# GuanRunwei/Achelous

Measured on AMD Instinct MI355X. Metric: frames/sec (whole node) EN-GDF-PN-S0 320x320+512pts bs64 @1/2/4/8 GPU, higher is better.
Workload: dtype bf16; 1 GPU; EN-GDF-PN-S0 forward + decode + NMS, 320x320 image + radar map, 512 points, batch 64 per GPU, all 5 heads, seeded random weights; radar_map=256 occupied cells per frame of 102 400 (SURVEY 8d: real maps are > 99 % zeros), global_batch=64, parallelism=batch-sharded x1, launches_per_forward=113

## Files before the change

achelous_amd/csrc/engine_impl.h:

```cpp
#pragma once
#include "engine.h"

#include <algorithm>
#include <cmath>
#include <cstring>

#include "k_dechead.h"
#include "k_csphead.h"
#include "k_upchain.h"
#include "k_detect.h"
#include "k_conv3.h"
#include "k_gemm.h"
#include "k_ghost.h"
#include "k_headdw.h"
#include "k_mlp.h"
#include "k_mlpband.h"
#include "k_mv2.h"
#include "k_mvit.h"
#include "k_nhwc.h"
#include "k_points.h"
#include "k_pn2.h"
#include "k_prepost.h"
#include "k_radar.h"
#include <functional>
#include "k_sdta.h"
#include "k_xca.h"
#include "k_xcaframe.h"

namespace ach {

#define ACH_HIP_CHECK(expr)                                                                               \
    do {                                                                                                  \
        hipError_t e_ = (expr);                                                                           \
        if (e_ != hipSuccess) throw AchError{ACH_ERR_DEVICE, std::string(#expr) + ": " + hipGetErrorString(e_)}; \
    } while (0)

static inline long round_up(long v, long m) { return (v + m - 1) / m * m; }

template <class T>
class Engine final : public EngineBase {
    using S = Store<T>;
    static constexpr int VEC = S::VEC;
    static constexpr int KC = 4 * VEC;
    static constexpr bool H16E = is_h16<T>::value;
    using IOB = typename std::conditional<std::is_same<T, f16_t>::value, bf16_t, T>::type;
    bool io_alt() const { return std::is_same<T, f16_t>::value && io_bf16; }

public:
    explicit Engine(const ach_config& c) : EngineBase(c) {}

    struct A {
        T* p = nullptr; int B = 0, H = 0, W = 0, C = 0; long ld = 0;
        long rows() const { return long(B) * H * W; }
        A slice(int c0, int c) const { A s = *this; s.p = p + c0; s.C = c; return s; }
    };
    struct Pl {
        T* p = nullptr; int B = 0, C = 0, H = 0, W = 0;
    };
    struct Lin { std::vector<float> w, b; int N = 0, K = 0; };

    A alloc(int B, int H, int W, int C) {
        A a; a.B = B; a.H = H; a.W = W; a.C = C; a.ld = round_up(C, 8);
        a.p = static_cast<T*>(aalloc(size_t(a.rows()) * a.ld * sizeof(T)));
        note_region(a.p, size_t(a.rows()) * a.ld * sizeof(T));
        return a;
    }
    A alloc_ld(int B, int H, int W, int C, long ld) {
        A a; a.B = B; a.H = H; a.W = W; a.C = C; a.ld = ld;
        a.p = static_cast<T*>(aalloc(size_t(a.rows()) * a.ld * sizeof(T)));
        note_region(a.p, size_t(a.rows()) * a.ld * sizeof(T));
        return a;
    }
    Pl alloc_pl(int B, int C, int H, int W) {
        Pl a; a.B = B; a.C = C; a.H = H; a.W = W;
        a.p = static_cast<T*>(aalloc(size_t(B) * C * H * W * sizeof(T)));
        note_region(a.p, size_t(B) * C * H * W * sizeof(T));
        return a;
    }
    float* alloc_f32(size_t n) { return static_cast<float*>(aalloc(n * sizeof(float))); }

    T* up_T(const std::vector<float>& v) {
        T* d = static_cast<T*>(walloc(v.size() * sizeof(T)));
        if (!measuring) {
            std::vector<T> h(v.size());
            for (size_t i = 0; i < v.size(); ++i) S::st(&h[i], v[i]);
            ACH_HIP_CHECK(hipMemcpy(d, h.data(), h.size() * sizeof(T), hipMemcpyHostToDevice));
        }
        return d;
    }
    void tap(const std::string& name, const A& a) {
        TapInfo t; t.ptr = a.p; t.kind = 0; t.B = a.B; t.H = a.H; t.W = a.W; t.C = a.C; t.ld = a.ld; add_tap(name, t);
    }
    void tap(const std::string& name, const Pl& a) {
        TapInfo t; t.ptr = a.p; t.kind = 1; t.B = a.B; t.H = a.H; t.W = a.W; t.C = a.C; add_tap(name, t);
    }

    Lin lin(const std::string& wkey, const std::string& bkey) const {
        const HostTensor& w = W(wkey);
        if (w.shape.size() < 2) throw AchError{ACH_ERR_MISSING_KEY, "not a matrix: " + wkey};
        Lin l; l.N = int(w.shape[0]); l.K = int(w.numel() / w.shape[0]);
        l.w = w.data;
        if (!bkey.empty() && hasW(bkey)) { l.b = W(bkey).data; if (int(l.b.size()) != l.N) throw AchError{ACH_ERR_MISSING_KEY, "bias shape: " + bkey}; }
        else l.b.assign(size_t(l.N), 0.f);
        return l;
    }
    void bn_coeffs(const std::string& pfx, double eps, std::vector<float>& scale, std::vector<float>& shift) const {
        const auto& g = W(pfx + ".weight").data; const auto& b = W(pfx + ".bias").data;
        const auto& m = W(pfx + ".running_mean").data; const auto& v = W(pfx + ".running_var").data;
        scale.resize(g.size()); shift.resize(g.size());
        for (size_t i = 0; i < g.size(); ++i) {
            const double s = double(g[i]) / std::sqrt(double(v[i]) + eps);
            scale[i] = float(s); shift[i] = float(double(b[i]) - double(m[i]) * s);
        }
    }
    void fold_bn(Lin& l, const std::string& pfx, double eps) const {
        std::vector<float> sc, sh; bn_coeffs(pfx, eps, sc, sh);
        if (int(sc.size()) != l.N) throw AchError{ACH_ERR_MISSING_KEY, "BatchNorm width mismatch at " + pfx};
        for (int n = 0; n < l.N; ++n) {
            for (int k = 0; k < l.K; ++k) l.w[size_t(n) * l.K + k] *= sc[n];
            l.b[n] = l.b[n] * sc[n] + sh[n];
        }
    }
    void fold_ln_in(Lin& l, const std::string& pfx) const {
        const auto& lw = W(pfx + ".weight").data; const auto& lb = W(pfx + ".bias").data;
        if (int(lw.size()) != l.K) throw AchError{ACH_ERR_MISSING_KEY, "LayerNorm width mismatch at " + pfx};
        for (int n = 0; n < l.N; ++n) {
            double acc = l.b[n];
            for (int k = 0; k < l.K; ++k) { acc += double(l.w[size_t(n) * l.K + k]) * lb[k]; l.w[size_t(n) * l.K + k] *= lw[k]; }
            l.b[n] = float(acc);
        }
    }
    void fold_scale_out(Lin& l, const std::vector<float>& g) const {
        for (int n = 0; n < l.N; ++n) { for (int k = 0; k < l.K; ++k) l.w[size_t(n) * l.K + k] *= g[n]; l.b[n] *= g[n]; }
    }

    std::vector<std::function<void()>> post_plan;
    struct Packed { T* w = nullptr; float* b = nullptr; int N = 0, K = 0, NT = 1, nchunks = 0, ksteps = 0; long group_elems = 0; };
    static int pick_nt(int N) { return N <= 16 ? 1 : (N <= 32 ? 2 : 4); }
    Packed pack_shape(int N, int K) const {
        Packed p; p.N = N; p.K = K; p.NT = pick_nt(N);
        p.nchunks = cdiv(N, 16 * p.NT); p.ksteps = cdiv(K, KC);
        p.group_elems = long(p.nchunks) * p.ksteps * p.NT * 64 * VEC;
        return p;
    }
    Packed pack(const Lin& l) {
        Packed p = pack_shape(l.N, l.K);
        std::vector<float> blob(size_t(p.group_elems), 0.f);
        if (!measuring)
            for (int n = 0; n < l.N; ++n)
                for (int k = 0; k < l.K; ++k) blob[size_t(wfrag_offset(n, k, p.NT, p.ksteps, VEC))] = l.w[size_t(n) * l.K + k];
        p.w = up_T(blob);
        p.b = up_f32(l.b);
        return p;
    }

    struct GemmOpt {
        int act = ACT_NONE; bool ln = false; float ln_eps = 0.f;
        bool ln_tap = false;
        const A* residual = nullptr;
        int conv_k = 0, conv_s = 1, conv_p = 0, Hin = 0, Win = 0, Cin = 0, Ho = 0, Wo = 0;
        int Creal = 0;
        void** ydyn = nullptr; int out_nchw = 0, HW = 0, Ctot = 0, coff = 0;
        int groups = 1; long w_group_stride = 0;
        const T* w_override = nullptr;
    };
    void gemm(const std::string& name, const T* Xp, long ldx, long M, const Packed& pk, T* Yp, long ldy, const GemmOpt& o) {
        GemmParams g;
        std::memset(&g, 0, sizeof(g));
        g.X = Xp; g.ldx = ldx; g.conv_k = o.conv_k; g.conv_s = o.conv_s; g.conv_p = o.conv_p; g.Hin = o.Hin; g.Win = o.Win; g.Cin = o.Cin; g.Ho = o.Ho; g.Wo = o.Wo;
        g.W = o.w_override ? o.w_override : pk.w; g.w_group_stride = o.w_group_stride;
        g.bias = pk.b; g.bias_group_stride = 0;
        g.Y = Yp; g.ldy = ldy;
        g.R = o.residual ? o.residual->p : nullptr; g.ldr = o.residual ? o.residual->ld : 0;
        g.groups = o.groups; g.M_per_group = int(M / o.groups);
        g.K = pk.K; g.N = pk.N; g.nchunks = pk.nchunks; g.ksteps = pk.ksteps;
        g.act = o.act; g.ln = o.ln_tap ? 2 : (o.ln ? 1 : 0); g.ln_eps = o.ln_eps;
        if (o.ln_tap && (o.conv_k != 2 || pk.NT != 4 || o.groups != 1 || batching || o.Cin % VEC != 0)) throw AchError{ACH_ERR_INVALID, name + ": per-tap LayerNorm needs a 2x2 conv with more than 32 outputs"};
        g.out_nchw = (o.out_nchw && io_alt()) ? 2 : o.out_nchw; g.HW = o.HW; g.Ctot = o.Ctot; g.coff = o.coff;
        g.vec_store = (ldy % 8 == 0 && (!o.residual || o.residual->ld % 8 == 0)) ? 1 : 0;
        if (ldx % VEC != 0) throw AchError{ACH_ERR_INVALID, name + ": activation row stride not 16-byte aligned"};
        if (o.conv_k > 0 && (o.Cin % VEC != 0 || pk.K != o.conv_k * o.conv_k * o.Cin)) throw AchError{ACH_ERR_UNSUPPORTED, name + ": conv channel count not 16-byte aligned"};
        const long kTargetBlocks = gemm_blocks > 0 ? gemm_blocks : 1024;
        int P = (!batching && pk.K >= 1024 && o.groups == 1 && gemm_rows > 1) ? gemm_rows : 1;
        while (P > 1 && cdivl(g.M_per_group, 64L * P) * pk.nchunks < 512) P >>= 1;
        const long row_blocks = cdivl(g.M_per_group, 64L * P) * g.groups;
        int zsplit = int(std::min<long>(pk.nchunks, std::max<long>(1, cdivl(kTargetBlocks, row_blocks))));
        g.chunks_per_block = cdiv(pk.nchunks, zsplit);
        const int NT = pk.NT;
        void** ydyn = o.ydyn;
        const double esz = double(sizeof(T));
        const double px_in = o.conv_k > 0 ? double(M) / (double(o.Ho) * o.Wo) * o.Hin * o.Win : 0.0;
        const double in_bytes = o.conv_k > 0 ? px_in * (o.Creal ? o.Creal : o.Cin) * esz : double(M) * pk.K * esz;
        const double rest = double(M) * pk.N * esz + (o.residual ? double(M) * pk.N * esz : 0.0)
                            + double(pk.group_elems) * esz * (o.w_group_stride ? o.groups : 1);
        const double bytes = in_bytes + rest;
        const double lbytes = (o.conv_k > 0 ? px_in * o.Cin * esz : in_bytes) + rest;
        if (batching) {
            if (g.groups != 1 || P != 1) throw AchError{ACH_ERR_INVALID, name + ": batched GEMMs must be ungrouped"};
            BatchJob j; j.kind = 0; j.name = name; j.g = g; j.NT = NT; j.ydyn = ydyn; j.bytes = bytes; j.flops = 2.0 * double(M) * (o.conv_k > 0 && o.Creal ? double(o.conv_k * o.conv_k * o.Creal) : double(pk.K)) * pk.N;
            batch_jobs.push_back(j);
            return;
        }
        add_op(name, [g, NT, P, ydyn](hipStream_t s) mutable {
            if (ydyn) g.Y = *ydyn;
            launch_gemm<T>(g, NT, P, s);
        }, bytes, 2.0 * double(M) * (o.conv_k > 0 && o.Creal ? double(o.conv_k * o.conv_k * o.Creal) : double(pk.K)) * pk.N, lbytes);
    }
    struct BatchJob { int kind = 0; std::string name; GemmParams g; int NT = 1; void** ydyn = nullptr; DwParams d; int ks = 0; double bytes = 0, flops = 0; HeadDwJob hj; int shared_in = 0; };
    bool batching = false;
    std::vector<BatchJob> batch_jobs;
    void flush_batch(int levels, int per_level) {
        batching = false;
        if (int(batch_jobs.size()) != levels * per_level || levels > 3) throw AchError{ACH_ERR_INVALID, "head batching: unexpected job count"};
        for (int st = 0; st < per_level; ++st) {
            const BatchJob& j0 = batch_jobs[size_t(st)];
            double bytes = 0, flops = 0;
            const std::string name = j0.name + "+levels";
            if (j0.kind == 0) {
                GemmJobs m;
                std::memset(&m, 0, sizeof(m));
                m.n = levels;
                unsigned gx = 1, gz = 1;
                void** yd[3] = {nullptr, nullptr, nullptr};
                for (int l = 0; l < levels; ++l) {
                    const BatchJob& j = batch_jobs[size_t(l * per_level + st)];
                    if (j.kind != 0 || j.NT != j0.NT) throw AchError{ACH_ERR_INVALID, "head batching: layer shapes differ across levels"};
                    m.p[l] = j.g;
                    m.nbx[l] = unsigned(cdivl(j.g.M_per_group, 64L));
                    m.nbz[l] = unsigned(cdiv(j.g.nchunks, j.g.chunks_per_block));
                    gx = std::max(gx, m.nbx[l]); gz = std::max(gz, m.nbz[l]);
                    yd[l] = j.ydyn; bytes += j.bytes; flops += j.flops;
                }
                const dim3 grid(gx, unsigned(levels), gz), block(256);
                const int NT = j0.NT;
                void** y0 = yd[0]; void** y1 = yd[1]; void** y2 = yd[2];
                add_op(name, [m, grid, block, NT, y0, y1, y2](hipStream_t s) mutable {
                    if (y0) m.p[0].Y = *y0;
                    if (y1) m.p[1].Y = *y1;
                    if (y2) m.p[2].Y = *y2;
                    if (NT == 1) ACH_LAUNCH((gemm_multi_kernel<T, 1>), grid, block, s, m);
                    else if (NT == 2) ACH_LAUNCH((gemm_multi_kernel<T, 2>), grid, block, s, m);
                    else ACH_LAUNCH((gemm_multi_kernel<T, 4>), grid, block, s, m);
                }, bytes, flops);
            } else if (j0.kind == 2) {
                HeadDwParams hp;
                std::memset(&hp, 0, sizeof(hp));
                hp.njobs = levels; hp.shared_in = j0.shared_in; hp.dbg = head_fuse_dbg;
                int wg = 0;
                for (int l = 0; l < levels; ++l) {
                    const BatchJob& j = batch_jobs[size_t(l * per_level + st)];
                    if (j.kind != 2 || j.shared_in != j0.shared_in) throw AchError{ACH_ERR_INVALID, "head batching: fused layers differ across levels"};
                    hp.job[l] = j.hj; hp.job[l].wg0 = wg;
                    hp.B = j.d.B;
                    wg += 2 * j.hj.bands * j.d.B;
                    bytes += j.bytes; flops += j.flops;
                }
                const dim3 grid(static_cast<unsigned>(wg)), block(HDW_THREADS);
                if constexpr (H16E)
                    add_op(name, [hp, grid, block](hipStream_t s) { ACH_LAUNCH((headdw_kernel<T>), grid, block, s, hp); }, bytes, flops);
                else throw AchError{ACH_ERR_INVALID, "head batching: the fused layer exists for 16-bit storage only"};
            } else {
                DwJobs m;
                std::memset(&m, 0, sizeof(m));
                m.n = levels;
                unsigned gx = 1;
                for (int l = 0; l < levels; ++l) {
                    const BatchJob& j = batch_jobs[size_t(l * per_level + st)];
                    if (j.kind != 1 || j.ks != 5 || j.d.stride != 1) throw AchError{ACH_ERR_INVALID, "head batching: depthwise shapes differ across levels"};
                    m.p[l] = j.d;
                    m.nbx[l] = unsigned(cdivl(long(j.d.B) * j.d.Ho * cdiv(j.d.Wo, 4) * (j.d.C / 4), 256));
                    gx = std::max(gx, m.nbx[l]);
                    bytes += j.bytes;
                }
                const dim3 grid(gx, unsigned(levels)), block(256);
                add_op(name, [m, grid, block](hipStream_t s) { ACH_LAUNCH((dwconv_strip_multi_kernel<T, 5, 4>), grid, block, s, m); }, bytes, 0);
            }
        }
        batch_jobs.clear();
    }
    void gemm(const std::string& name, const A& X, const Packed& pk, const A& Y, const GemmOpt& o = GemmOpt()) {
        gemm(name, X.p, X.ld, X.rows(), pk, Y.p, Y.ld, o);
    }

    void dwconv(const std::string& name, const A& X, const A* X2, const std::string& wkey, const std::string& bkey,
                const std::string& bnpfx, double bneps, int ks, int stride, int act, const A& Y) {
        const HostTensor& w = W(wkey);
        const int C = X.C;
        if (w.shape[0] != C || w.numel() != long(C) * ks * ks) throw AchError{ACH_ERR_MISSING_KEY, "depthwise weight shape: " + wkey};
        if (C % 4) throw AchError{ACH_ERR_UNSUPPORTED, name + ": depthwise channel count must be a multiple of 4"};
        std::vector<float> wt(size_t(ks) * ks * C), bias(size_t(C), 0.f), sc(size_t(C), 1.f), sh(size_t(C), 0.f);
        if (!bkey.empty()) bias = W(bkey).data;
        if (!bnpfx.empty()) bn_coeffs(bnpfx, bneps, sc, sh);
        for (int c = 0; c < C; ++c) {
            for (int t = 0; t < ks * ks; ++t) wt[size_t(t) * C + c] = w.data[size_t(c) * ks * ks + t] * sc[c];
            bias[c] = bias[c] * sc[c] + sh[c];
        }
        if (double(X.rows()) * double(std::max(X.ld, X2 ? X2->ld : 0L)) * sizeof(T) >= 2147483648.0)
            throw AchError{ACH_ERR_UNSUPPORTED, name + ": depthwise input of 2 GiB or more (batch too large for one plan)"};
        DwParams p;
        std::memset(&p, 0, sizeof(p));
        p.X = X.p; p.ldx = X.ld; p.X2 = X2 ? X2->p : nullptr; p.ldx2 = X2 ? X2->ld : 0;
        p.W = up_f32(wt); p.bias = up_f32(bias); p.Y = Y.p; p.ldy = Y.ld;
        p.B = X.B; p.H = X.H; p.Wd = X.W; p.C = C; p.Ho = Y.H; p.Wo = Y.W; p.stride = stride; p.act = act;
        p.tile = (dw_tile && X.H * X.W <= 144) ? 1 : 0;
        const double px_in = double(X.B) * X.H * X.W * C * sizeof(T), px_out = double(Y.B) * Y.H * Y.W * C * sizeof(T);
        add_op(name, [p, ks](hipStream_t s) { launch_dwconv<T>(p, ks, s); }, px_in * (X2 ? 2 : 1) + px_out, 0);
    }

    template <class K, class Pm>
    void ew(const std::string& name, K kern, const Pm& p, long total, double bytes = 0, double layout_bytes = -1) {
        const dim3 grid(unsigned(cdivl(total, 256))), block(256);
        add_op(name, [kern, p, grid, block](hipStream_t s) { ACH_LAUNCH(kern, grid, block, s, p); }, bytes, 0, layout_bytes);
    }
    void add(const std::string& name, const A& a, const A& b, const A& y) {
        AddParams p{a.p, a.ld, b.p, b.ld, y.p, y.ld, a.rows(), a.C};
        ew(name, add_kernel<T>, p, a.rows() * (a.C / 4), 3.0 * a.rows() * a.C * sizeof(T));
    }
    void copy(const std::string& name, const A& x, const A& y, const float* posenc = nullptr) {
        CopyParams p{x.p, x.ld, y.p, y.ld, x.rows(), x.C, posenc, x.H * x.W};
        ew(name, copy_kernel<T>, p, x.rows() * (x.C / 4), 2.0 * x.rows() * x.C * sizeof(T));
    }
    int stats(const std::string& name, const A& x, float*& partial) {
        const int HW = x.H * x.W;
        const int S = HW >= 1024 ? 8 : (HW >= 256 ? 4 : 1);
        partial = alloc_f32(size_t(x.B) * S * 2 * x.C);
        StatParams p{x.p, x.ld, partial, HW, x.C, S};
        const dim3 grid(unsigned(x.B), unsigned(S)), block(256);
        add_op(name, [p, grid, block](hipStream_t s) { ACH_LAUNCH(chan_stats_kernel<T>, grid, block, s, p); });
        return S;
    }

    struct EnCfg { int depths[4]; int dims[4]; int heads; int scales[4]; int ks[4]; };
    EnCfg en_cfg() const {
        switch (cfg.phi) {
            case ACH_PHI_S0: return {{2, 2, 6, 2}, {32, 48, 96, 176}, 4, {2, 2, 3, 4}, {3, 5, 7, 9}};
            case ACH_PHI_S1: return {{3, 3, 9, 3}, {32, 48, 120, 224}, 4, {2, 2, 3, 4}, {3, 5, 7, 9}};
            default: return {{3, 3, 9, 3}, {32, 64, 144, 288}, 8, {2, 2, 3, 4}, {3, 5, 7, 9}};
        }
    }
    float* posenc_table(const std::string& pfx, int H, int Wd, int C) {
        const int hidden = 32;
        const HostTensor& w = W(pfx + ".token_projection.weight");
        const HostTensor& b = W(pfx + ".token_projection.bias");
        std::vector<float> tab(size_t(H) * Wd * C);
        if (!measuring) {
            std::vector<float> feat(2 * hidden);
            for (int y = 0; y < H; ++y)
                for (int x = 0; x < Wd; ++x) {
                    const float ye = float(y + 1) / (float(H) + 1e-6f) * float(2.0 * M_PI);
                    const float xe = float(x + 1) / (float(Wd) + 1e-6f) * float(2.0 * M_PI);
                    for (int i = 0; i < hidden; ++i) {
                        const float dim_t = std::pow(10000.0f, float(2 * (i / 2)) / float(hidden));
                        const float py = ye / dim_t, px = xe / dim_t;
                        feat[i] = (i % 2 == 0) ? std::sin(py) : std::cos(py);
                        feat[hidden + i] = (i % 2 == 0) ? std::sin(px) : std::cos(px);
                    }
                    for (int c = 0; c < C; ++c) {
                        double acc = b.data[c];
                        for (int k = 0; k < 2 * hidden; ++k) acc += double(w.data[size_t(c) * 2 * hidden + k]) * feat[k];
                        tab[(size_t(y) * Wd + x) * C + c] = float(acc);
                    }
                }
        }
        return up_f32(tab);
    }

    A pw_mlp(const std::string& pfx, const A& xin, const A& resid) {
        const int C = xin.C;
        Lin l1 = lin(pfx + ".pwconv1.weight", pfx + ".pwconv1.bias");
        fold_ln_in(l1, pfx + ".norm");
        Lin l2 = lin(pfx + ".pwconv2.weight", pfx + ".pwconv2.bias");
        fold_scale_out(l2, W(pfx + ".gamma").data);
        A h = alloc(xin.B, xin.H, xin.W, 4 * C);
        GemmOpt o1; o1.act = ACT_GELU; o1.ln = true; o1.ln_eps = 1e-6f;
        gemm(pfx + ".pwconv1", xin, pack(l1), h, o1);
        A y = block_out(xin);
        GemmOpt o2; o2.residual = &resid;
        gemm(pfx + ".pwconv2", h, pack(l2), y, o2);
        return y;
    }
    struct BandOp { size_t op; MlpBandParams bp; int nb, shape; };
    std::vector<BandOp> band_ops;
    void merge_band_runs() {
#if !defined(ACH_HOSTEMU)
        if constexpr (H16E) {
            if (measuring || !mlp_band_run || use_graph) { band_ops.clear(); return; }
            for (size_t a = 0; a < band_ops.size();) {
                size_t e = a + 1;
                while (e < band_ops.size() && e - a < size_t(MLPB_RUN_MAX) && band_ops[e].op == band_ops[e - 1].op + 1 && band_ops[e].shape == band_ops[a].shape && band_ops[e].nb == band_ops[a].nb &&
                       band_ops[e].bp.m.X == band_ops[e - 1].bp.m.Y && band_ops[e].bp.bands == band_ops[a].bp.bands && band_ops[e].bp.rb == band_ops[a].bp.rb &&
                       ops[band_ops[e].op].stream == ops[band_ops[a].op].stream && !ops[band_ops[e].op].wait && !ops[band_ops[e].op].xwait &&
                       !ops[band_ops[e - 1].op].signal && !ops[band_ops[e - 1].op].xsignal) ++e;
                const size_t n = e - a;
                const long nwg = long(band_ops[a].bp.bands) * band_ops[a].nb;
                if (n >= 2 && mlp_band_run_shape(band_ops[a].shape) && nwg % 8 == 0 && (nwg / 8) % band_ops[a].bp.bands == 0) {
                    MlpBandRunParams rp;
                    std::memset(&rp, 0, sizeof(rp));
                    for (size_t k = 0; k < n; ++k) rp.blk[k] = band_ops[a + k].bp;
                    rp.n = int(n);
                    std::vector<unsigned> zeros(size_t(band_ops[a].nb), 0u);
                    rp.sync = static_cast<unsigned*>(up_raw(zeros.data(), zeros.size() * sizeof(unsigned)));
                    const int nb = band_ops[a].nb, shape = band_ops[a].shape;
                    const size_t first = band_ops[a].op, last = band_ops[e - 1].op;
                    Op& op = ops[first];
                    for (size_t k = first + 1; k <= last; ++k) { op.bytes += ops[k].bytes; op.layout_bytes += ops[k].layout_bytes; op.flops += ops[k].flops; }
                    op.signal = ops[last].signal; op.xsignal = ops[last].xsignal;
                    op.name += "..+" + std::to_string(n - 1);
                    op.fn = [rp, nb, shape](hipStream_t s) mutable { launch_mlp_band_run<T>(rp, shape, nb, s); ++rp.epoch; };
                    ops.erase(ops.begin() + long(first) + 1, ops.begin() + long(last) + 1);
                    for (size_t k = e; k < band_ops.size(); ++k) band_ops[k].op -= n - 1;
                }
                a = e;
            }
        }
#endif
        band_ops.clear();
    }
    bool fused_mlp(const std::string& pfx, const A& xin, const A& resid, int dw_ks, A& y) {
        if (!fuse_mlp || mlp_pick_dt(xin.C) == 0) return false;
        Lin l1 = lin(pfx + ".pwconv1.weight", pfx + ".pwconv1.bias");
        fold_ln_in(l1, pfx + ".norm");
        Lin l2 = lin(pfx + ".pwconv2.weight", pfx + ".pwconv2.bias");
        fold_scale_out(l2, W(pfx + ".gamma").data);
        return fused_mlp_lin(pfx + (dw_ks ? ".block" : ".mlp"), pfx, xin, resid, dw_ks, l1, l2, ACT_GELU, 1e-6f, y);
    }
    A preset_out; bool has_preset = false;
    A block_out(const A& like) {
        if (has_preset) {
            has_preset = false;
            reached(kPtConcatSlice);
            if (preset_out.B != like.B || preset_out.H != like.H || preset_out.W != like.W || preset_out.C != like.C)
                throw AchError{ACH_ERR_INVALID, "preset block output does not match the block"};
            return preset_out;
        }
        return alloc(like.B, like.H, like.W, like.C);
    }
    bool fused_mlp_lin(const std::string& name, const std::string& pfx, const A& xin, const A& resid, int dw_ks, const Lin& l1, const Lin& l2,
                       int act, float ln_eps, A& y) {
        if (!fuse_mlp) return false;
        const int C = xin.C, DT = mlp_pick_dt(C);
        if (DT == 0 || (dw_ks != 0 && dw_ks != 3 && dw_ks != 5 && dw_ks != 7 && dw_ks != 9)) return false;
        const int hidden = l1.N, k1 = cdiv(C, KC), J = cdiv(hidden, 32), hstep = 8 / VEC, ks2 = J * hstep;
        if (l1.K != C || l2.N != C || l2.K != hidden) throw AchError{ACH_ERR_MISSING_KEY, "MLP shapes at " + pfx};
        std::vector<float> w1(size_t(J) * k1 * 2 * 64 * VEC, 0.f), b1(size_t(J) * 32, 0.f);
        std::vector<float> w2(size_t(ks2) * DT * 64 * VEC, 0.f), b2(size_t(DT) * 16, 0.f);
        if (!measuring) {
            for (int n = 0; n < hidden; ++n) {
                b1[n] = l1.b[n];
                for (int k = 0; k < C; ++k) w1[size_t(wfrag_offset(n, k, 2, k1, VEC))] = l1.w[size_t(n) * C + k];
            }
            for (int n = 0; n < C; ++n) {
                b2[n] = l2.b[n];
                for (int kap = 0; kap < 32 * J; ++kap) {
                    const int ch = mlp_hidden_channel(kap, VEC);
                    if (ch < hidden) w2[size_t(wfrag_offset(n, kap, DT, ks2, VEC))] = l2.w[size_t(n) * hidden + ch];
                }
            }
        }
        MlpParams mp;
        std::memset(&mp, 0, sizeof(mp));
        mp.X = xin.p; mp.ldx = xin.ld; mp.R = resid.p; mp.ldr = resid.ld;
        y = block_out(xin);
        mp.Y = y.p; mp.ldy = y.ld;
        mp.dw_k = dw_ks; mp.H = xin.H; mp.W = xin.W;
        if (dw_ks) {
            const double xb = double(xin.rows()) * double(xin.ld) * sizeof(T);
            if (xb >= 2147483648.0) throw AchError{ACH_ERR_UNSUPPORTED, "depthwise input of 2 GiB or more (batch too large for one plan)"};
            mp.xbytes = unsigned(xb);
        }
        if (dw_ks) {
            const HostTensor& w = W(pfx + ".dwconv.weight");
            const std::vector<float>& b = W(pfx + ".dwconv.bias").data;
            const int ldc = k1 * KC, kk = dw_ks * dw_ks;
            if (size_t(w.numel()) != size_t(C) * size_t(kk)) throw AchError{ACH_ERR_MISSING_KEY, "depthwise shape at " + pfx};
            std::vector<float> wt(size_t(kk) * ldc, 0.f), bt(size_t(ldc), 0.f);
            for (int c = 0; c < C; ++c) { bt[c] = b[c]; for (int t = 0; t < kk; ++t) wt[size_t(t) * ldc + c] = w.data[size_t(c) * kk + t]; }
            mp.Wdw = up_f32(wt); mp.bdw = up_f32(bt);
        }
        mp.W1 = up_T(w1); mp.b1 = up_f32(b1); mp.W2 = up_T(w2); mp.b2 = up_f32(b2);
        mp.M = xin.rows(); mp.C = C; mp.k1 = k1; mp.J = J; mp.act = act; mp.ln_eps = ln_eps; mp.ln = 1; mp.Cout = C;
        const bool split = mlp_split < 0 ? xin.H * xin.W <= mlp_split_hw : mlp_split != 0;
        if (split && dw_ks && dw_even && mlp_even_dt(DT)) {
            const int U = k1 * dw_ks, chunk = cdiv(U, 4);
            bool ok = chunk < cdiv(k1, 4) * dw_ks;
            for (int w = 0; w < 4 && ok; ++w) {
                const int u0 = w * chunk, u1 = std::min(U, u0 + chunk);
                if (u0 < u1 && (u1 - 1) / dw_ks > u0 / dw_ks + 1) ok = false;
            }
            mp.dw_even = ok ? 1 : 0;
        }
        const double bytes = double(mp.M) * C * sizeof(T) * (xin.p == resid.p ? 2.0 : 3.0);
        const double flops = 4.0 * double(mp.M) * C * hidden + (dw_ks ? 2.0 * double(mp.M) * C * dw_ks * dw_ks : 0.0);
        if constexpr (H16E) if (mlp_band && (split || mlp_band > 1) && dw_ks && act == ACT_GELU && xin.p == resid.p && mlp_band_supported(k1, DT, dw_ks, xin.H, xin.W)) {
            MlpBandParams bp;
            bp.m = mp; bp.rb = mlp_band_rows(k1, DT, dw_ks, xin.H, xin.W);
            if (band_rows_s3 > 0 && mlp_band_shape(k1, DT, dw_ks, xin.W) == 2) bp.rb = std::min(std::min(band_rows_s3, 5), xin.H);
            bp.bands = cdiv(xin.H, bp.rb); bp.dbg = mlp_band_dbg;
            int shape = mlp_band_shape(k1, DT, dw_ks, xin.W);
            if (shape == 1 && mlp_band_lean) shape = 11;
            const int nb = xin.B;
            if (!measuring) band_ops.push_back(BandOp{ops.size(), bp, nb, shape});
            add_op(name, [bp, nb, shape](hipStream_t s) { launch_mlp_band<T>(bp, shape, nb, s); }, bytes, flops);
            return true;
        }
        if constexpr (H16E) if (ffn_rows2 && !split && !dw_ks && (DT == 10 || DT == 12)) {
            add_op(name, [mp, DT](hipStream_t s) { launch_ffn2<T>(mp, DT, s); }, bytes, flops);
            return true;
        }
// ... 1808 lines not shown
```

Before: 39980 frames/s.

## Add specialized LayerNorm-fused GEMM kernel normalizing each row once

Adds a dedicated kernel for LayerNorm-prefixed GEMMs (plain or per-tap for 2x2 stride convs) that loads and normalizes each row's input once in registers, then iterates over all output chunks with a pipelined weight prefetch. When several chunks exist, a multi-wave block shares the normalized row via LDS so each wave computes different output chunks. This is meant to avoid recomputing the LayerNorm statistics per output tile or z-split block. It only covers a fixed set of K values for 16-bit types with NT=4, and may lose parallelism compared with the z-split generic path.

```diff
diff --git a/achelous_amd/csrc/engine_impl.h b/achelous_amd/csrc/engine_impl.h
--- a/achelous_amd/csrc/engine_impl.h
+++ b/achelous_amd/csrc/engine_impl.h
@@ -11,6 +11,7 @@
 #include "k_detect.h"
 #include "k_conv3.h"
 #include "k_gemm.h"
+#include "k_lngemm.h"
 #include "k_ghost.h"
 #include "k_headdw.h"
 #include "k_mlp.h"
@@ -201,9 +202,12 @@
             batch_jobs.push_back(j);
             return;
         }
-        add_op(name, [g, NT, P, ydyn](hipStream_t s) mutable {
+        const bool rows_once = H16E && NT == 4 && P == 1 && (o.ln || o.ln_tap) && ln_gemm_rows_has<T>(pk.K, o.ln_tap) &&
+                               (o.ln_tap ? (o.conv_k == 2 && pk.K == 4 * o.Cin) : o.conv_k == 0);
+        add_op(name, [g, NT, P, ydyn, rows_once](hipStream_t s) mutable {
             if (ydyn) g.Y = *ydyn;
-            launch_gemm<T>(g, NT, P, s);
+            if (rows_once) launch_ln_gemm_rows<T>(g, s);
+            else launch_gemm<T>(g, NT, P, s);
         }, bytes, 2.0 * double(M) * (o.conv_k > 0 && o.Creal ? double(o.conv_k * o.conv_k * o.Creal) : double(pk.K)) * pk.N, lbytes);
     }
     struct BatchJob { int kind = 0; std::string name; GemmParams g; int NT = 1; void** ydyn = nullptr; DwParams d; int ks = 0; double bytes = 0, flops = 0; HeadDwJob hj; int shared_in = 0; };
diff --git a/achelous_amd/csrc/k_lngemm.h b/achelous_amd/csrc/k_lngemm.h
--- /dev/null
+++ b/achelous_amd/csrc/k_lngemm.h
@@ -0,0 +1,231 @@
+#pragma once
+#include "k_gemm.h"
+
+namespace ach {
+
+template <class T, int NT>
+__device__ __forceinline__ void ln_gemm_store_tile(const GemmParams& p, const f32x4 (&acc)[NT], const float (&bv)[4 * NT], long m, int cbase, int g) {
+    float o[4 * NT];
+    ACH_UNROLL
+    for (int t = 0; t < NT; ++t)
+        ACH_UNROLL
+        for (int r = 0; r < 4; ++r) o[t * 4 + r] = acc[t][r] + bv[t * 4 + r];
+    apply_act_n<T, 4 * NT>(o, p.act);
+    if (p.out_nchw) {
+        T* Y = static_cast<T*>(p.Y);
+        const long b = m / p.HW, pix = m - b * p.HW;
+        ACH_UNROLL
+        for (int t = 0; t < NT; ++t)
+            ACH_UNROLL
+            for (int r = 0; r < 4; ++r) {
+                const int n = cbase + chunk_channel(NT, t, g, r);
+                if (n < p.N) st_user<T>(Y, (b * p.Ctot + p.coff + n) * p.HW + pix, o[t * 4 + r], p.out_nchw == 2);
+            }
+        return;
+    }
+    T* yrow = static_cast<T*>(p.Y) + m * p.ldy;
+    const T* rrow = p.R ? static_cast<const T*>(p.R) + m * p.ldr : nullptr;
+    static_assert(NT >= 2, "pairs of 16-channel tiles");
+    ACH_UNROLL
+    for (int j = 0; j < NT / 2; ++j) {
+        const int nb = cbase + j * 32 + g * 8;
+        if (nb >= p.N) continue;
+        float v8[8];
+        ACH_UNROLL
+        for (int i = 0; i < 8; ++i) v8[i] = o[j * 8 + i];
+        if (p.vec_store && nb + 8 <= p.N) {
+            if (rrow) { float r8[8]; Store<T>::ld8(rrow + nb, r8); ACH_UNROLL for (int i = 0; i < 8; ++i) v8[i] += r8[i]; }
+            Store<T>::st8(yrow + nb, v8);
+        } else {
+            for (int i = 0; i < 8; ++i)
+                if (nb + i < p.N) {
+                    float v = v8[i];
+                    if (rrow) v += Store<T>::ld(rrow + nb + i);
+                    Store<T>::st(yrow + nb + i, v);
+                }
+        }
+    }
+}
+
+constexpr int LNG_DEPTH = 3;
+constexpr int LNG_MAX_WAVES = 10;
+
+template <class T, int K, bool LNTAP>
+__device__ __forceinline__ void ln_rows_phase_a(const GemmParams& p, bool valid, long m, int g, uint4 (&xr)[(K + 4 * Store<T>::VEC - 1) / (4 * Store<T>::VEC)]) {
+    constexpr int VEC = Store<T>::VEC, KC = 4 * VEC, KS = (K + KC - 1) / KC, CIN = K / 4;
+    static_assert(!LNTAP || (K % KC == 0 && CIN % VEC == 0), "per-tap LayerNorm: whole k-steps, a lane's channels inside one tap");
+    const T* X = static_cast<const T*>(p.X);
+    long xbase = m * p.ldx;
+    int iy0 = 0, ix0 = 0;
+    if constexpr (LNTAP) {
+        const long b = m / (long(p.Ho) * p.Wo);
+        const int rem = int(m - b * long(p.Ho) * p.Wo);
+        const int oy = rem / p.Wo, ox = rem - oy * p.Wo;
+        iy0 = oy * p.conv_s - p.conv_p;
+        ix0 = ox * p.conv_s - p.conv_p;
+        xbase = b * p.Hin * long(p.Win);
+    }
+    ACH_UNROLL
+    for (int s = 0; s < KS; ++s) {
+        const int k0 = s * KC + g * VEC;
+        xr[s] = make_uint4(0u, 0u, 0u, 0u);
+        if (!valid || k0 >= K) continue;
+        if constexpr (LNTAP) {
+            const int tap = k0 / CIN, c = k0 - tap * CIN;
+            const int iy = iy0 + (tap >> 1), ix = ix0 + (tap & 1);
+            if (iy < 0 || iy >= p.Hin || ix < 0 || ix >= p.Win) continue;
+            xr[s] = *reinterpret_cast<const uint4*>(X + (xbase + long(iy) * p.Win + ix) * p.ldx + c);
+        } else {
+            xr[s] = *reinterpret_cast<const uint4*>(X + xbase + k0);
+        }
+    }
+    if constexpr (LNTAP) {
+        float s1[4] = {0.f, 0.f, 0.f, 0.f}, s2[4] = {0.f, 0.f, 0.f, 0.f};
+        ACH_UNROLL
+        for (int s = 0; s < KS; ++s) {
+            float v[8];
+            frag_unpack<T>(xr[s], v);
+            float a1 = 0.f, a2 = 0.f;
+            ACH_UNROLL
+            for (int j = 0; j < VEC; ++j) { a1 += v[j]; a2 += v[j] * v[j]; }
+            const int tp = (s * KC + g * VEC) / CIN;
+            ACH_UNROLL
+            for (int t = 0; t < 4; ++t) { s1[t] += tp == t ? a1 : 0.f; s2[t] += tp == t ? a2 : 0.f; }
+        }
+        float tmean[4], trstd[4];
+        ACH_UNROLL
+        for (int t = 0; t < 4; ++t) {
+            s1[t] += __shfl_xor(s1[t], 16); s2[t] += __shfl_xor(s2[t], 16);
+            s1[t] += __shfl_xor(s1[t], 32); s2[t] += __shfl_xor(s2[t], 32);
+            const float mu = s1[t] / float(CIN);
+            float var = s2[t] / float(CIN) - mu * mu;
+            var = var > 0.f ? var : 0.f;
+            tmean[t] = mu;
+            trstd[t] = ln_rstd(var + p.ln_eps);
+        }
+        ACH_UNROLL
+        for (int s = 0; s < KS; ++s) {
+            const int tp = (s * KC + g * VEC) / CIN;
+            const float mu = tp == 0 ? tmean[0] : (tp == 1 ? tmean[1] : (tp == 2 ? tmean[2] : tmean[3]));
+            const float rs = tp == 0 ? trstd[0] : (tp == 1 ? trstd[1] : (tp == 2 ? trstd[2] : trstd[3]));
+            float v[8];
+            frag_unpack<T>(xr[s], v);
+            ACH_UNROLL
+            for (int j = 0; j < VEC; ++j) v[j] = (v[j] - mu) * rs;
+            xr[s] = frag_pack<T>(v);
+        }
+    } else {
+        float s1 = 0.f, s2 = 0.f;
+        ACH_UNROLL
+        for (int s = 0; s < KS; ++s) {
+            float v[8];
+            frag_unpack<T>(xr[s], v);
+            ACH_UNROLL
+            for (int j = 0; j < VEC; ++j) { s1 += v[j]; s2 += v[j] * v[j]; }
+        }
+        s1 += __shfl_xor(s1, 16); s2 += __shfl_xor(s2, 16);
+        s1 += __shfl_xor(s1, 32); s2 += __shfl_xor(s2, 32);
+        const float mean = s1 / float(K);
+        float var = s2 / float(K) - mean * mean;
+        var = var > 0.f ? var : 0.f;
+        const float rstd = ln_rstd(var + p.ln_eps);
+        ACH_UNROLL
+        for (int s = 0; s < KS; ++s) {
+            float v[8];
+            frag_unpack<T>(xr[s], v);
+            ACH_UNROLL
+            for (int j = 0; j < VEC; ++j) v[j] = (v[j] - mean) * rstd;
+            xr[s] = frag_pack<T>(v);
+        }
+    }
+}
+
+template <class T, int K, bool LNTAP, bool SHARE>
+__global__ __launch_bounds__(SHARE ? 64 * LNG_MAX_WAVES : 256) void ln_gemm_rows_kernel(const GemmParams p) { f16_sat_mode<T>();
+    constexpr int NT = 4, VEC = Store<T>::VEC, KC = 4 * VEC, KS = (K + KC - 1) / KC;
+    constexpr int DEPTH = KS < LNG_DEPTH ? KS : LNG_DEPTH;
+    __shared__ __attribute__((aligned(16))) uint4 xs[SHARE ? KS * 64 : 1];
+    const int lane = threadIdx.x & 63, wave = wave_uniform(int(threadIdx.x >> 6));
+    const int px = lane & 15, g = lane >> 4;
+    const int grp = blockIdx.y;
+    const long row0 = SHARE ? long(blockIdx.x) * 16 : long(LNTAP ? xcd_block(blockIdx.x, gridDim.x) : blockIdx.x) * 64 + wave * 16;
+    const long mloc = row0 + px;
+    const bool valid = mloc < p.M_per_group;
+    const long m = long(grp) * p.M_per_group + (valid ? mloc : 0);
+    const uint4* Wf = reinterpret_cast<const uint4*>(static_cast<const T*>(p.W) + long(grp) * p.w_group_stride) + lane;
+    const float* bias = p.bias + long(grp) * p.bias_group_stride;
+
+    int c0, cstep, c_end;
+    if constexpr (SHARE) { c0 = wave; cstep = int(blockDim.x >> 6); c_end = p.nchunks; }
+    else { c0 = int(blockIdx.z) * p.chunks_per_block; cstep = 1; c_end = (c0 + p.chunks_per_block < p.nchunks) ? c0 + p.chunks_per_block : p.nchunks; }
+
+    uint4 wb[DEPTH][NT];
+    auto fill = [&](int d, int c, int s) {
+        ACH_UNROLL
+        for (int t = 0; t < NT; ++t) wb[d][t] = Wf[((long(c) * KS + s) * NT + t) * 64];
+    };
+    uint4 xr[KS];
+    if constexpr (SHARE) {
+        if (wave == 0) {
+            ln_rows_phase_a<T, K, LNTAP>(p, valid, m, g, xr);
+            ACH_UNROLL
+            for (int s = 0; s < KS; ++s) xs[s * 64 + lane] = xr[s];
+        }
+        ACH_UNROLL
+        for (int d = 0; d < DEPTH; ++d) fill(d, c0, d);
+        __syncthreads();
+    } else {
+        ln_rows_phase_a<T, K, LNTAP>(p, valid, m, g, xr);
+        if (c0 < c_end) {
+            ACH_UNROLL
+            for (int d = 0; d < DEPTH; ++d) fill(d, c0, d);
+        }
+    }
+
+    for (int c = c0; c < c_end; c += cstep) {
+        const int cbase = c * (16 * NT);
+        float bv[4 * NT];
+        ACH_UNROLL
+        for (int t = 0; t < NT; ++t) {
+            const f32x4 b4 = *reinterpret_cast<const f32x4*>(bias + cbase + chunk_channel(NT, t, g, 0));
+            bv[t * 4] = b4[0]; bv[t * 4 + 1] = b4[1]; bv[t * 4 + 2] = b4[2]; bv[t * 4 + 3] = b4[3];
+        }
+        f32x4 acc[NT];
+        ACH_UNROLL
+        for (int t = 0; t < NT; ++t) { acc[t][0] = 0.f; acc[t][1] = 0.f; acc[t][2] = 0.f; acc[t][3] = 0.f; }
+        const int cn = c + cstep;
+        ACH_UNROLL
+        for (int s = 0; s < KS; ++s) {
+            const int d = s % DEPTH;
+            uint4 xf;
+            if constexpr (SHARE) xf = xs[s * 64 + lane]; else xf = xr[s];
+            ACH_UNROLL
+            for (int t = 0; t < NT; ++t) mfma16<T>(wb[d][t], xf, acc[t]);
+            if (s + DEPTH < KS) fill(d, c, s + DEPTH);
+            else if (cn < c_end) fill(d, cn, s + DEPTH - KS);
+        }
+        if (valid) ln_gemm_store_tile<T, NT>(p, acc, bv, m, cbase, g);
+    }
+}
+
+template <class T> inline bool ln_gemm_rows_has(int K, bool tap) {
+    if constexpr (!is_h16<T>::value) return false;
+    return tap ? (K == 128 || K == 192 || K == 384) : (K == 48 || K == 96 || K == 176);
+}
+template <class T>
+inline void launch_ln_gemm_rows(const GemmParams& p, hipStream_t stream) {
+    if constexpr (is_h16<T>::value) {
+        const int nw = cdiv(p.nchunks, p.chunks_per_block) < LNG_MAX_WAVES ? cdiv(p.nchunks, p.chunks_per_block) : LNG_MAX_WAVES;
+        const bool share = nw > 1;
+        const dim3 grid(unsigned(cdivl(p.M_per_group, share ? 16L : 64L)), unsigned(p.groups), 1u), block(share ? 64u * unsigned(nw) : 256u);
+#define ACH_LNG_CASE(k, tap) if (p.K == k && (p.ln == 2) == tap) { \
+            if (share) ACH_LAUNCH((ln_gemm_rows_kernel<T, k, tap, true>), grid, block, stream, p); \
+            else ACH_LAUNCH((ln_gemm_rows_kernel<T, k, tap, false>), grid, block, stream, p); \
+            return; }
+        ACH_LNG_CASE(128, true) ACH_LNG_CASE(192, true) ACH_LNG_CASE(384, true)
+        ACH_LNG_CASE(48, false) ACH_LNG_CASE(96, false) ACH_LNG_CASE(176, false)
+#undef ACH_LNG_CASE
+    }
+}
+
+}
```

New measurement: 40620 frames/s (median of 6 runs). 1.02x the previous value.
